# nathancunn/ParticleMDI.jl

Hardware: AMD Instinct MI355X
Metric: Gibbs iters/sec (and obs·particles/sec) at 1/2/4/8 GPUs vs CPU ref (higher is better)
Workload: dtype f64

## Files before the change

### particlemdi.jl_amd/csrc/pmdi_sweep2_body.h

```cpp
#pragma once
#include "pmdi_arith.h"
#include "pmdi_internal.h"
#include "pmdi_sweep2_layout.h"

#ifndef PM2_LANE_API_PROVIDED
#include "pmdi_wave.h"
#define PM2_DEV __device__ __forceinline__
#define PM2_COLD __device__ __noinline__
extern __shared__ __attribute__((aligned(16))) unsigned char pm2_smem_[];
#define PM2_SMEM (pm2_smem_)
#define PM2_TID() ((int)threadIdx.x)
#define PM2_BID() ((int)blockIdx.x)
#define PM2_BALLOT(p) __ballot(p)
#define PM2_SHFL64(v, src) pm2_shfl64((v), (src))
#define PM2_WAVE_BARRIER() do { __builtin_amdgcn_fence(__ATOMIC_ACQ_REL, "wavefront"); __builtin_amdgcn_wave_barrier(); } while (0)
#define PM2_BARRIER() __syncthreads()
#define PM2_LDS_BARRIER() asm volatile("s_waitcnt lgkmcnt(0)\n\ts_barrier" ::: "memory")
#define PM2_UNI(x) __builtin_amdgcn_readfirstlane(x)
#define PM2_CLOCK() ((long long)clock64())
#define PM2_WALLCLOCK() ((long long)wall_clock64())
#if defined(__HIP_DEVICE_COMPILE__)
#define PM2_G(T, p) ((__attribute__((address_space(1))) T *)(p))
#define PM2_CONST __attribute__((address_space(4)))
#ifdef PM2_NO_LAUNDER
// ... 931 lines not shown
                u64 wm0 = readlane_u64(wm, l0);
                const int base0 = readlane_i(base, l0), inpl0 = readlane_i(inpl, l0);
                int rnk = 0;
                while (wm0) {
                    const int ns = pm2_ffs64(wm0) - 1;
                    wm0 &= wm0 - 1;
                    if (ns != inpl0) {
                        const int newc = base0 + rnk - (inpl0 >= 0 ? 1 : 0);
                        const int t = v.tgt_get(v.tab_get(cs, ns));
                        if (lane < N) v.tab_set(newc, lane, lane == ns ? t : v.tab_get(cs, lane));
                    }
                    rnk += 1;
                }
                PM2_WAVE_BARRIER();
                if (inpl0 >= 0 && lane == 0) v.tab_set(cs, inpl0, v.tgt_get(v.tab_get(cs, inpl0)));
                if (lane == l0) todo = false;
            }
            }
            ncol_new += tot;
        }
        PM2_WAVE_BARRIER();
        PHC(6);
        unsigned mpr_r = INFU;
        int slot_r = 0;
        if (nk <= 64) {
            const u64 repb = PM2_BALLOT(rep_r);
            for (u64 rb = repb; rb; rb &= rb - 1) {
                const int j2 = pm2_ffs64(rb) - 1;
                const int v2 = readlane_i(kv_r, j2);
                const unsigned m2 = (unsigned)readlane_i((int)mp_r, j2);
                if (v2 == kv_r) mpr_r = m2;
            }
            for (u64 rb = repb; rb; rb &= rb - 1) {
                const int j2 = pm2_ffs64(rb) - 1;
                const unsigned m2 = (unsigned)readlane_i((int)mp_r, j2);
                if (m2 < mpr_r) ++slot_r;
            }
        }
        for (int j0 = 0; j0 < nk; j0 += 64) {
            const int j = j0 + lane;
            if (j < nk) {
                const int key = klist[j];
                const int v0 = kval[j];
                unsigned mpr = mpr_r;
                int slot = slot_r;
                if (nk > 64) {
                    int jr = j;
                    for (int j2 = 0; j2 < nk; ++j2) if (krep[j2] && kval[j2] == v0) jr = j2;
                    mpr = minp[klist[jr]];
                    slot = 0;
                    for (int j2 = 0; j2 < nk; ++j2) if (krep[j2] && minp[klist[j2]] < mpr) ++slot;
                }
                lds<u8>(v.base + L.knew)[key] = (u8)slot;
                if (krep[j]) {
                    const int pl = (int)(mpr >> 16), cl = (int)(mpr & 0xffffu);
                    const int ns = key - (key / N) * N;
                    const u64 wm = nclone ? v.wmask_get(cl) : 0ull;
                    int newc = cl;
                    if ((wm >> ns) & 1ull) {
                        const int bi = v.cbi_get(cl);
                        const int inpl = (bi & 0xff) - 1, base = bi >> 8;
                        const int rnk = pm2_popc64(wm & ((1ull << ns) - 1ull));
                        newc = (inpl >= 0) ? (ns == inpl ? cl : base + rnk - 1) : base + rnk;
                    }
                    lds<int>(v.base + L.clsval)[slot] = v0; lds<int>(v.base + L.clslead)[slot] = pl; lds<int>(v.base + L.leadcol)[slot] = newc;
                }
            }
        }
        PM2_WAVE_BARRIER();
        PHD(13);
        PHC(7);
        int ndefer = 0;
        {
            const bool on = lane < D && fl[lane];
            for (int e0 = 0; e0 < nd; e0 += 4) {
                int cj[4], nj[4], sj[4];
                bool mine[4];
                St stj[4];
                double gj[4];
#pragma unroll
                for (int j = 0; j < 4; ++j) {
                    cj[j] = 0; nj[j] = 0; sj[j] = NONE8; mine[j] = false;
                    if (e0 + j < nd) {
                        cj[j] = chosen(e0 + j);
                        sj[j] = v.slot_of(cj[j]);
                        mine[j] = sj[j] != NONE8 && v.tgt_get(cj[j]) == cj[j];
                        if (mine[j]) nj[j] = v.cn_get(cj[j]); else ndefer += 1;
                    }
                }
#pragma unroll
                for (int j = 0; j < 4; ++j) {
                    stj[j] = pf; gj[j] = 0.0;
                    if (mine[j]) {
                        if (e0 + j > 0) stj[j] = st_load(v, cj[j], x, lane < D);
                        if (lane == 0 && (GO || v.kind == K_GAUSSIAN)) gj[j] = PM2_G(const double, d.gtab)[nj[j]];
                    }
                }
#pragma unroll
                for (int j = 0; j < 4; ++j) {
                    if (mine[j]) {
                        st_add_store(v, cj[j], stj[j], x, nj[j], on);
                        cache_fill(v, k, sj[j], stj[j].a, stj[j].b, nj[j], false, true, gj[j]);
                    }
                }
            }
        }
        PHD(15);
        PHC(8);
        PM2_WAVE_BARRIER();
        for (int e0 = 0; e0 < nd; e0 += 64) {
            const int e = e0 + lane;
            if (e < nd) { const int c = chosen(e); v.ncop_set(c, 0); v.firstp_set(c, 0x7fffffff); }
        }
        for (int j0 = 0; j0 < nk; j0 += 64) { const int j = j0 + lane; if (j < nk) minp[klist[j]] = INFU; }
        for (int w = lane; w < P / 64 + 1; w += 64) { bmc[w] = 0; bmf[w] = 0; }
        if (lane == 0) {
            long long *st = stat();
            pm2_atomic_add((u64 *)&st[0], (u64)maxid);
            pm2_atomic_add((u64 *)&st[4], (u64)ncls);
            pm2_atomic_add((u64 *)&st[2], (u64)nclone);
            pm2_atomic_add((u64 *)&st[5], (u64)1);
            pm2_atomic_max((u64 *)&st[3], (u64)(maxid + nclone));
            long long *w_ = wk(k);
            w_[WK_EVAL] += dsc[DS_NNEED]; w_[WK_UPD] += nd; w_[WK_CLONE] += nclone; w_[WK_SPLITS] += ncol_new - ncol;
            dsc[DS_MAXID] = maxid + nclone; dsc[DS_NCLS] = nrep; dsc[DS_NCOL] = ncol_new; dsc[DS_NDX] = 0; dsc[DS_NCLONE] = nclone;
            dsc[DS_ND] = ndefer ? nd : 0; dsc[DS_NDLOW] = nd_low;
            dsc[DS_FOLLOW] = (nclone != 0 || ncls != 1 || nk != 1) ? 1 : 0;
            dsc[DS_DIRTY] = (nclone != 0 || ncls != 1 || nk != 1 || dsc[DS_CHANGED] != 0) ? 1 : 0;
            dsc[DS_CHANGED] = 0;
        }
        (void)pos;
        return true;
    }

    PM2_DEV bool help_stats(int i_cur)
    {
        constexpr int HB = 2;
        int item = 0;
        bool any = false;
#pragma nounroll
        for (int k = 0; k < K; ++k) {
            const DV v = view(k);
            const int *dsc = v.dsc();
            const int nd = PM2_UNI(dsc[DS_ND]);
            if (nd == 0) continue;
            any = true;
            const int nd_low = PM2_UNI(dsc[DS_NDLOW]);
            const auto &d = ap->ds[k];
            const int D = d.D;
            const u8 *fl = flk(k);
            const bool on = lane < D && fl[lane];
            const u16 *clist = lds<u16>(v.base + L.clist);
            auto sb = PM2_G(double, v.ar.sb());
            double x = 0.0;
            bool have_x = false;
            for (int e0 = 0; e0 < nd; e0 += HB, ++item) {
                if (item % NW != wave) continue;
                if (!have_x) { x = obs_x(k, i_cur); have_x = true; }
                int cj[HB], tj[HB], nj[HB];
                bool mine[HB];
                double sgj[HB], btj[HB];
#pragma unroll
                for (int j = 0; j < HB; ++j) {
                    cj[j] = 0; tj[j] = 0; nj[j] = 0; mine[j] = false;
                    if (e0 + j < nd) {
                        const int e = e0 + j;
                        cj[j] = (e < nd_low) ? (int)clist[e] : PM2_G(const int, v.ar.dl())[e - nd_low];
                        tj[j] = v.tgt_get(cj[j]);
                        mine[j] = !(v.slot_of(cj[j]) != NONE8 && tj[j] == cj[j]);
                        if (mine[j]) nj[j] = v.cn_get(tj[j]);
                    }
                }
                if ((GO || v.kind == K_GAUSSIAN)) {
#pragma unroll
                    for (int j = 0; j < HB; ++j) {
                        sgj[j] = 0.0; btj[j] = 0.5;
                        if (mine[j] && lane < D) { sgj[j] = sb[((size_t)cj[j] * D + lane) * 2]; btj[j] = sb[((size_t)cj[j] * D + lane) * 2 + 1]; }
                    }
#pragma unroll
                    for (int j = 0; j < HB; ++j) {
                        if (mine[j]) {
                            double sg = sgj[j], bt = btj[j];
                            if (on) pmdi_arith::gauss_add_sb(x, nj[j], sg, bt);
                            if (lane < D && (on || tj[j] != cj[j])) { sb[((size_t)tj[j] * D + lane) * 2] = sg; sb[((size_t)tj[j] * D + lane) * 2 + 1] = bt; }
                        }
                    }
                } else if ((!GO && v.kind == K_CATEGORICAL)) {
                    auto cn_ = PM2_G(int, v.ar.cnt());
                    const int Lc = v.Lc;
#pragma unroll
                    for (int j = 0; j < HB; ++j) {
                        if (mine[j] && lane < D) {
                            const size_t so = ((size_t)cj[j] * D + lane) * Lc, to = ((size_t)tj[j] * D + lane) * Lc;
                            const int xl = (int)x - 1;
                            const int cx = cn_[so + xl];
                            if (tj[j] != cj[j]) for (int l = 0; l < Lc; ++l) cn_[to + l] = cn_[so + l];
                            if (on) cn_[to + xl] = cx + 1;
                        }
                    }
                } else {
                    auto nb_ = PM2_G(long long, v.ar.nbs());
#pragma unroll
                    for (int j = 0; j < HB; ++j)
                        if (mine[j] && lane < D && (on || tj[j] != cj[j]))
                            nb_[(size_t)tj[j] * D + lane] = nb_[(size_t)cj[j] * D + lane] + (on ? (long long)x : 0ll);
                }
            }
        }
        return any;
    }

    PM2_DEV void census(const DV &v, bool active, int mult, int r, int cl, int ns, int c, int p)
    {
        int *dsc = v.dsc();
        const int key3 = ((r * P + cl) * N + ns) * 16 + mult;
        const u64 act = PM2_BALLOT(active);
        if (act == 0) return;
        const int l0 = pm2_ffs64(act) - 1;
        const int k0 = readlane_i(key3, l0);
        const bool uni = PM2_BALLOT(active && key3 == k0) == act;
        if (uni ? (lane == l0) : active) {
            const int cnt = uni ? pm2_popc64(act) * mult : mult;
            if (c < v.idcap) {
                pm2_atomic_add(lds<int>(v.base + L.ncop) + c, cnt);
                pm2_atomic_min(lds<int>(v.base + L.firstp) + c, p);
                pm2_atomic_or(lds<u64>(v.base + L.cbm) + (c >> 6), 1ull << (c & 63));
            } else {
                const int old = pm2_atomic_min(v.ar.firstp() + c, p);
                pm2_atomic_add(v.ar.ncop() + c, cnt);
                if (old == 0x7fffffff) { const int idx = pm2_atomic_add(&dsc[DS_NDX], 1); PM2_G(int, v.ar.dl())[idx] = c; }
            }
            const int key = r * N + ns;
            pm2_atomic_min(&lds<unsigned>(v.base + L.minp)[key], ((unsigned)p << 16) | (unsigned)cl);
            pm2_atomic_or(lds<u64>(v.base + L.kbm) + (key >> 6), 1ull << (key & 63));
            v.cmask_or(cl, 1ull << ns);
        }
    }

    PM2_DEV void cumsum_pairwise(const double (&w)[PPL], double (&c)[PPL])
    {
        constexpr int LPB = 64 / PPL;
        double sl[PPL];
#pragma unroll
        for (int u = 0; u < PPL; ++u) sl[u] = 0.0;
        const int blk = (tid * PPL) >> 6;
        const int lib = tid % LPB;
        double *tot = lds<double>(L.leaf_tot), *car = lds<double>(L.leaf_carry);
        double acc = 0.0;
        for (int pass = 0; pass < 2; ++pass) {
            const bool mine = (pass == 0) ? (blk != 1) : (blk == 1);
            double carry_in = 0.0;
            if (pass == 1) carry_in = tot[0];
            for (int t = 0; t < LPB; ++t) {
                const double cin = prev_lane_d(acc);
                if (mine && lib == t) {
                    double s = (t == 0) ? carry_in : cin;
#pragma unroll
                    for (int u = 0; u < PPL; ++u) {
                        const int p = tid * PPL + u;
                        if (p == 0) continue;
                        const bool first = (p == 1) || ((p & 63) == 0 && p >= 128);
                        s = first ? w[u] : s + w[u];
                        sl[u] = s;
                    }
                    acc = s;
                }
            }
            if (mine && lib == LPB - 1) tot[blk] = acc;
            PM2_BARRIER();
        }
        const int nb = P >> 6;
        double *lv = car;
        if (wave == 0) {
            if (tid == 0) lds<double>(L.red)[121] = w[0];
            for (int h = 1; (nb >> h) >= 2; ++h) {
                const int cnt = nb >> h, off = nb - (nb >> (h - 1)), offp = (h >= 2) ? nb - (nb >> (h - 2)) : 0;
                if (lane < cnt) {
                    double val;
                    if (h == 1) val = (lane == 0) ? tot[1] : tot[2 * lane] + tot[2 * lane + 1];
                    else val = lv[offp + 2 * lane] + lv[offp + 2 * lane + 1];
                    lv[off + lane] = val;
                }
                PM2_WAVE_BARRIER();
            }
        }
        PM2_BARRIER();
        double carry = lds<double>(L.red)[121];
        if (blk >= 2) {
            const int j = 32 - __builtin_clz((unsigned)blk);
            carry = carry + lv[nb - (nb >> (j - 2))];
            for (int h = j - 2; h >= 0; --h)
                if ((blk >> h) & 1) {
                    const int g = (blk >> h) - 1;
                    carry = carry + (h == 0 ? tot[g] : lv[nb - (nb >> (h - 1)) + g]);
                }
        }
#pragma unroll
        for (int u = 0; u < PPL; ++u) {
            const int p = tid * PPL + u;
            c[u] = (p == 0) ? w[u] : carry + sl[u];
        }
    }

    PM2_DEV void resample(long long pos, double mx)
    {
        PHR(0);
        double w[PPL];
#pragma unroll
        for (int u = 0; u < PPL; ++u) w[u] = exp(lw[u] - mx);
        const double u01 = pmdi_arith::uniform01<false>(seed, iter, (unsigned)pos, 0, 0, SITE_RESAMPLE_U);
        const double usl = pmdi_arith::uniform01<false>(seed, iter, (unsigned)pos, 0, 0, SITE_RESAMPLE_SLOT);
        double c[PPL];
        PHR(1);
        cumsum_pairwise(w, c);
        PHR(2);
        double *utab = lds<double>(L.tr);
        u16 *jtab = lds<u16>(L.tr + L.rs_jtab), *raw = lds<u16>(L.tr + L.rs_raw), *anc = lds<u16>(L.tr + L.rs_anc);
        double *red = lds<double>(L.red);
        if (tid == T - 1) red[0] = c[PPL - 1];
        {
            const double h = 1.0 / (double)P;
            const int j = tid * PPL;
            double u = pmdi_arith::resample_u_at(u01, P, j);
#pragma unroll
            for (int uu = 0; uu < PPL; ++uu) { utab[j + uu] = u; u = u + h; }
        }
        PM2_BARRIER();
        PHR(3);
        {
            const double last = red[0];
#pragma unroll
            for (int uu = 0; uu < PPL; ++uu) {
                const double q = c[uu] / last;
                int J = (int)((q - utab[0]) * (double)P) + 1;
                if (J < 0) J = 0;
                if (J > P) J = P;
                while (J < P && q >= utab[J]) ++J;
                while (J > 0 && !(q >= utab[J - 1])) --J;
                jtab[tid * PPL + uu] = (u16)J;
            }
        }
        PM2_BARRIER();
        PHR(4);
        {
            int lo = 0;
#pragma unroll
            for (int uu = 0; uu < PPL; ++uu) {
                const int j = tid * PPL + uu;
                if (uu == 0 || !((int)jtab[lo] > j)) {
                    int hi = P - 1;
                    while (lo < hi) { const int mid = (lo + hi) >> 1; if ((int)jtab[mid] > j) hi = mid; else lo = mid + 1; }
                }
                raw[j] = (u16)lo;
            }
        }
        int js = (int)(usl * (double)P);
        if (js >= P) js = P - 1;
        PM2_BARRIER();
        PHR(5);
#pragma unroll
        for (int uu = 0; uu < PPL; ++uu) {
            const int p = tid * PPL + uu;
            anc[p] = (p == 0) ? (u16)0 : (p <= js ? raw[p - 1] : raw[p]);
            lw.set(uu, 1.0);
        }
        PM2_BARRIER();
        u16 *scol = lds<u16>(L.tr), *mult = lds<u16>(L.tr + P * 2), *cmap = lds<u16>(L.tr + P * 4);
        u8 *scsl = lds<u8>(L.tr + P * 6);
        int *hist = lds<int>(L.tr + L.rs_hist);
#pragma nounroll
        for (int k = 0; k < K; ++k) {
            const DV v = view(k);
            int *dsc = v.dsc();
            const int ncol_old = dsc[DS_NCOL], oldmax = dsc[DS_MAXID], ncls_old = dsc[DS_NCLS];
            PHR(6);
            int ck[PPL], rk[PPL];
            col_get(k, ck);
#pragma unroll
            for (int uu = 0; uu < PPL; ++uu) rk[uu] = csl_get(k, uu);
#pragma unroll
            for (int uu = 0; uu < PPL; ++uu) { const int p = tid * PPL + uu; scol[p] = (u16)ck[uu]; scsl[p] = (u8)rk[uu]; }
            for (int e = tid; e < ncol_old; e += T) mult[e] = 0;
            for (int e = tid; e <= oldmax && e < v.idcap; e += T) hist[e] = 0;
            if (tid < CLSMAX) lds<int>(L.red)[RI_CLSMIN + tid] = 0x7fffffff;
            if (tid == 0) sc()[SC_TMP0] = 0;
            PM2_BARRIER();
#pragma unroll
            for (int uu = 0; uu < PPL; ++uu) {
                const int p = tid * PPL + uu;
                const int an = anc[p];
                ck[uu] = scol[an]; rk[uu] = scsl[an];
            }
            PHR(7);
#pragma unroll
            for (int uu = 0; uu < PPL; ++uu) {
                const int cl = ck[uu], r = rk[uu];
                bool start = true;
                if (uu > 0) start = cl != ck[uu - 1] || r != rk[uu - 1];
                int cnt = 1;
                {
                    bool go = true;
#pragma unroll
                    for (int u2 = uu + 1; u2 < PPL; ++u2) { go = go && ck[u2] == cl && rk[u2] == r; cnt += go ? 1 : 0; }
                }
                const u64 act = PM2_BALLOT(start);
                if (act) {
                    const int l0 = pm2_ffs64(act) - 1;
                    const int key = cl * CLSMAX + r;
                    const int key0 = readlane_i(key, l0);
                    const bool uni = PM2_BALLOT(start && key == key0) == act;
                    int tot = cnt;
                    if (uni) {
                        tot = 0;
#pragma unroll
                        for (int c_ = 1; c_ <= PPL; ++c_) tot += c_ * pm2_popc64(PM2_BALLOT(start && cnt == c_));
                    }
                    if (uni ? (lane == l0) : start) {
                        pm2_atomic_add((unsigned *)mult + (cl >> 1), (unsigned)tot << ((cl & 1) * 16));
                        pm2_atomic_min(&lds<int>(L.red)[RI_CLSMIN + r], tid * PPL + uu);
                    }
                }
            }
            PM2_BARRIER();
            PHR(8);
            int ncol_new = 0;
            for (int b = 0; b < ncol_old; b += T) {
                const int cc = b + tid;
                const bool live = cc < ncol_old && mult[cc] != 0;
                const u64 bal = PM2_BALLOT(live);
                if (lane == 0) lds<int>(L.red)[RI_WCNT + wave] = pm2_popc64(bal);
                PM2_BARRIER();
                int basew = ncol_new, tot = 0;
                for (int w_ = 0; w_ < T / 64; ++w_) { const int cnt = lds<int>(L.red)[RI_WCNT + w_]; if (w_ < wave) basew += cnt; tot += cnt; }
                if (live) cmap[cc] = (u16)(basew + pm2_popc64(bal & ((1ull << lane) - 1ull)));
                ncol_new += tot;
                PM2_BARRIER();
            }
            PHR(9);
            for (int idx = tid; idx < ncol_old * N; idx += T) {
                const int cc = idx / N;
                const int m = mult[cc];
                if (m) {
                    const int id = v.tab_get(cc, idx - cc * N);
                    if (id < v.idcap) pm2_atomic_add(&hist[id], m); else pm2_atomic_add(v.ar.ncop() + id, m);
                }
            }
            PM2_BARRIER();
            PHR(10);
            int newmax = 0;
            for (int b = 0; b < oldmax; b += T) {
                const int id = 1 + b + tid;
                int occ = 0;
                if (id <= oldmax) occ = (id < v.idcap) ? hist[id] : PM2_G(int, v.ar.ncop())[id];
                const bool live = occ != 0;
                const u64 bal = PM2_BALLOT(live);
                if (lane == 0) lds<int>(L.red)[RI_WCNT + wave] = pm2_popc64(bal);
                PM2_BARRIER();
                int basew = newmax, tot = 0;
                for (int w_ = 0; w_ < T / 64; ++w_) { const int cnt = lds<int>(L.red)[RI_WCNT + w_]; if (w_ < wave) basew += cnt; tot += cnt; }
                if (id <= oldmax) v.tgt_set(id, live ? basew + pm2_popc64(bal & ((1ull << lane) - 1ull)) + 1 : 0);
                newmax += tot;
                PM2_BARRIER();
            }
            PHR(11);
            for (int b = 0; b < oldmax; b += T) {
                const int id = 1 + b + tid;
                int nid = 0, occ = 0, cnv = 0;
                if (id <= oldmax) {
                    nid = v.tgt_get(id);
                    occ = (id < v.idcap) ? hist[id] : PM2_G(int, v.ar.ncop())[id];
                    cnv = v.cn_get(id);
                    if (id >= v.idcap) PM2_G(int, v.ar.ncop())[id] = 0;
                }
                {
                    const u64 mvb = PM2_BALLOT(nid != 0 && nid != id);
                    if (lane == 0 && mvb) pm2_atomic_add(&sc()[SC_TMP0], pm2_popc64(mvb));
                }
                PM2_BARRIER();
                if (id <= oldmax) {
                    if (nid) { v.counts_set(nid, occ); v.cn_set(nid, cnv); }
                    if (id > newmax) v.counts_set(id, 0);
                }
                PM2_BARRIER();
            }
            PHR(12);
            if (sc()[SC_TMP0] != 0) {
                const int D = ap->ds[k].D;
                if ((GO || v.kind == K_GAUSSIAN)) {
                    auto sb = PM2_G(double, v.ar.sb());
                    const long long nitems = (long long)oldmax * D;
                    for (long long b = 0; b < nitems; b += T) {
                        const long long it = b + tid;
                        const int id = 1 + (int)(it / D), q = (int)(it - (long long)(id - 1) * D);
                        const int nid = (it < nitems) ? v.tgt_get(id) : 0;
                        const bool mv = nid != 0 && nid != id;
                        double sg = 0.0, bt = 0.0;
                        if (mv) { sg = sb[((size_t)id * D + q) * 2]; bt = sb[((size_t)id * D + q) * 2 + 1]; }
                        PM2_BARRIER();
                        if (mv) { sb[((size_t)nid * D + q) * 2] = sg; sb[((size_t)nid * D + q) * 2 + 1] = bt; }
                    }
                } else if ((!GO && v.kind == K_CATEGORICAL)) {
                    auto cn_ = PM2_G(int, v.ar.cnt());
                    const int W = D * v.Lc;
                    const long long nitems = (long long)oldmax * W;
                    for (long long b = 0; b < nitems; b += T) {
                        const long long it = b + tid;
                        const int id = 1 + (int)(it / W), q = (int)(it - (long long)(id - 1) * W);
                        const int nid = (it < nitems) ? v.tgt_get(id) : 0;
                        const bool mv = nid != 0 && nid != id;
                        int c_ = 0;
                        if (mv) c_ = cn_[(size_t)id * W + q];
                        PM2_BARRIER();
                        if (mv) cn_[(size_t)nid * W + q] = c_;
                    }
                } else {
                    auto nb_ = PM2_G(long long, v.ar.nbs());
                    const long long nitems = (long long)oldmax * D;
                    for (long long b = 0; b < nitems; b += T) {
                        const long long it = b + tid;
                        const int id = 1 + (int)(it / D), q = (int)(it - (long long)(id - 1) * D);
                        const int nid = (it < nitems) ? v.tgt_get(id) : 0;
                        const bool mv = nid != 0 && nid != id;
                        long long S_ = 0;
                        if (mv) S_ = nb_[(size_t)id * D + q];
                        PM2_BARRIER();
                        if (mv) nb_[(size_t)nid * D + q] = S_;
                    }
                }
            }
            PM2_BARRIER();
            PHR(13);
            if (wave == k) {
                int *slot_id = lds<int>(v.base + L.slot_id);
                int olds = 0, news = 0;
                if (lane < NS) { olds = slot_id[lane]; news = olds ? v.tgt_get(olds) : 0; }
                PM2_WAVE_BARRIER();
                if (lane < NS && olds) v.slot_set(olds, NONE8);
                PM2_WAVE_BARRIER();
                if (lane < NS) { slot_id[lane] = news; if (news) v.slot_set(news, lane); }
            }
            {
                const int cpr = (2 * T) / N;
                for (int c0 = 0; c0 < ncol_old; c0 += cpr) {
                    int nv[2], dc[2], dn[2];
#pragma unroll
                    for (int h = 0; h < 2; ++h) {
                        const int idx = h * T + tid;
                        const int cc = c0 + idx / N, nn = idx - (idx / N) * N;
                        nv[h] = 0; dc[h] = -1; dn[h] = nn;
                        if (idx < cpr * N && cc < ncol_old && mult[cc] != 0) { nv[h] = v.tgt_get(v.tab_get(cc, nn)); dc[h] = cmap[cc]; }
                    }
                    PM2_BARRIER();
#pragma unroll
                    for (int h = 0; h < 2; ++h) if (dc[h] >= 0) v.tab_set(dc[h], dn[h], nv[h]);
                    PM2_BARRIER();
                }
            }
#pragma unroll
            for (int uu = 0; uu < PPL; ++uu) ck[uu] = cmap[ck[uu]];
            {
                int *redi = lds<int>(L.red);
                int nc2 = 0;
                for (int r = 0; r < ncls_old; ++r) nc2 += (redi[RI_CLSMIN + r] != 0x7fffffff) ? 1 : 0;
                if (tid < ncls_old) {
                    int s = 0;
                    const int mine = redi[RI_CLSMIN + tid];
                    for (int r2 = 0; r2 < ncls_old; ++r2) if (redi[RI_CLSMIN + r2] < mine) ++s;
                    redi[RI_NEWSLOT + tid] = s;
                    redi[RI_CLSVAL + tid] = lds<int>(v.base + L.clsval)[tid];
                }
                PM2_BARRIER();
#pragma unroll
                for (int uu = 0; uu < PPL; ++uu) {
                    const int p = tid * PPL + uu;
                    const int r = rk[uu];
                    const int ns_ = redi[RI_NEWSLOT + r];
                    rk[uu] = ns_;
                    if (redi[RI_CLSMIN + r] == p) {
                        lds<int>(v.base + L.clsval)[ns_] = redi[RI_CLSVAL + r]; lds<int>(v.base + L.clslead)[ns_] = p; lds<int>(v.base + L.leadcol)[ns_] = ck[uu];
                    }
                }
                col_put(k, ck);
#pragma unroll
                for (int uu = 0; uu < PPL; ++uu) csl_put(k, uu, rk[uu]);
                if (tid == 0) {
                    const int moved = sc()[SC_TMP0];
                    dsc[DS_NCLS] = nc2; dsc[DS_NCOL] = ncol_new; dsc[DS_MAXID] = newmax; dsc[DS_DIRTY] = 1;
                    long long *w_ = wk(k);
                    w_[WK_COLS] += ncol_old; w_[WK_MOVED] += moved; w_[WK_MOVE_EVENTS] += moved ? 1 : 0;
                }
            }
            PM2_BARRIER();
        }
        PHR(15);
    }

    PM2_DEV void run(const SweepArgs *ap_, int chain_)
    {
        ap = (const PM2_CONST SweepArgs *)ap_; chain = chain_;
        const auto &a = *ap;
        tid = PM2_TID(); lane = tid & 63; wave = tid >> 6;
        N = a.N; P = a.P; n = a.n; n1 = a.n1; iter = a.iter;
        seed = a.seed + (unsigned long long)chain;
        const long long t_start = PM2_CLOCK();
        const long long t_wall = a.phase ? PM2_WALLCLOCK() : 0ll;
        const bool owner = wave < K;
        auto order = PM2_G(const int, a.order) + (size_t)chain * n;
        auto logphi = PM2_G(const double, a.logphi) + (size_t)chain * a.npairs;
        if (tid < SC_COUNT) sc()[tid] = 0;
        if (tid < 8) stat()[tid] = 0;
        if (tid < KMAX2 * 8) lds<long long>(L.wk)[tid] = 0;
        if (tid < 16) lds<long long>(L.ph)[tid] = 0;
        long long ph_last = 0;
        int ph_cur = 0;
#ifdef PM2_DETAIL_TIMERS
        phd_last = PM2_CLOCK(); phd_cur = 15;
#define PH2(i_) do { } while (0)
#else
#define PH2(i_) do { if (a.phase && tid == 0) { const long long t_ = PM2_CLOCK(); lds<long long>(L.ph)[ph_cur] += t_ - ph_last; ph_last = t_; ph_cur = (i_); } } while (0)
#endif
        if (a.phase && tid == 0) ph_last = PM2_CLOCK();
        PM2_BARRIER();
#pragma unroll
        for (int u = 0; u < PPL; ++u) lw.set(u, a.lw_init);
#pragma unroll
        for (int k = 0; k < K; ++k)
#pragma unroll
            for (int j = 0; j < NCP; ++j) colp.set(k * NCP + j, 0u);
#pragma unroll
        for (int k = 0; k < NCSW; ++k) cslp.set(k, (csl_t)0);
#pragma unroll
        for (int s = 0; s < NS; ++s) { c_mu.set(s, 0.0); c_lam.set(s, 1.0); }
        PM2_BARRIER();
        if (owner) prefix(wave);
        PM2_BARRIER();
        PH2(1);

        double xnext = 0.0;
        int ns0_next = 0;
        int i_next = order[n1 - 1];
        int i_next2 = (n1 < n) ? order[n1] : 0;
        if (owner) {
            xnext = obs_x(wave, i_next);
            ns0_next = PM2_G(const int, a.s_in)[((size_t)chain * K + wave) * n + i_next];
        }
        pend_slot = -1; pend_g = 0.0;
        int failed = 0, handed = 0;
        long long pos_handed = 0;
        for (long long pos = n1 - 1; pos < n; ++pos) {
            PM2_LAUNDER(ap, SweepArgs);
            PM2_FRESH_VGPR(tid); PM2_FRESH_VGPR(lane);
            const double x = xnext;
            const int ns0_cur = ns0_next;
            const int i_cur = i_next;
            if (pos + 1 < n) {
                i_next = i_next2;
                if (owner) {
                    xnext = obs_x(wave, i_next);
                    ns0_next = PM2_G(const int, a.s_in)[((size_t)chain * K + wave) * n + i_next];
                }
                if (pos + 2 < n) i_next2 = order[pos + 2];
            }
            PH2(1);
            if (owner) phase_a(wave, x, ns0_cur, pos);
            PH2(2);
            PM2_BARRIER();
            PH2(3);
            if (sc()[SC_FAIL]) { failed = sc()[SC_FAIL]; break; }
            unsigned nsp[PPL];
#pragma unroll
            for (int u = 0; u < PPL; ++u) nsp[u] = 0;
#pragma nounroll
            for (int k = 0; k < K; ++k) {
                const DV v = view(k);
                const int ns0 = v.dsc()[DS_NS0];
                PHD(5);
                int cl_[PPL], r_[PPL], c_[PPL];
                RegArr<int, PPL> nsv;
                double inc_[PPL];
                bool draw_any = false;
#pragma unroll
                for (int u = 0; u < PPL; ++u) {
                    const int p = tid * PPL + u;
                    r_[u] = csl_get(k, u);
                    cl_[u] = (int)((colp[k * NCP + (u >> 1)] >> ((u & 1) * 16)) & 0xffffu);
                    const int hot = (int)cdf_get(v, r_[u], N + 1);
                    inc_[u] = cdf_get(v, r_[u], N);
                    const int ns = (p == 0) ? ns0 : hot;
                    nsv.set(u, ns);
                    draw_any |= ns < 0;
                }
                PHD(6);
                if (PM2_BALLOT(draw_any)) {
#pragma nounroll
                    for (int u = 0; u < PPL; ++u) {
                        if (nsv[u] < 0) {
                            const int p = tid * PPL + u;
                            const int rr = csl_get(k, u);
                            const double u01 = pmdi_arith::uniform01<false>(seed, iter, (unsigned)pos, (unsigned)k, (unsigned)p, SITE_DRAW);
                            int ns = 0, t = 0;
                            if (!CDFA || rr < v.cdfl) {
                                const double *row = v.cdf_row_l(rr);
                                for (; t + 4 <= N - 1; t += 4) {
                                    const double a0 = row[t], a1 = row[t + 1], a2 = row[t + 2], a3 = row[t + 3];
                                    ns += ((a0 > u01) ? 0 : 1) + ((a1 > u01) ? 0 : 1) + ((a2 > u01) ? 0 : 1) + ((a3 > u01) ? 0 : 1);
                                }
                                for (; t < N - 1; ++t) ns += (row[t] > u01) ? 0 : 1;
                            } else {
                                auto row = PM2_G(const double, v.ar.cdfg()) + (size_t)rr * (N + 2);
                                for (; t < N - 1; ++t) ns += (row[t] > u01) ? 0 : 1;
                            }
                            nsv.set(u, ns);
                        }
                    }
                }
                PHD(7);
                unsigned packed = 0;
#pragma unroll
                for (int u = 0; u < PPL; ++u) {
                    const int ns = nsv[u];
                    lw.set(u, lw[u] + inc_[u]);
                    c_[u] = v.tab_get(cl_[u], ns);
                    nsp[u] |= (unsigned)ns << (8 * k);
                    packed |= (unsigned)ns << (8 * (u & 3));
                    if ((u & 3) == 3 || u == PPL - 1) {
                        u8 *ss = v.ar.sstar() + (size_t)pos * P + (size_t)tid * PPL + (u & ~3);
                        if (PPL >= 4) *PM2_G(unsigned, ss) = packed;
                        else if (PPL == 2) *PM2_G(u16, ss) = (u16)packed;
                        else *PM2_G(u8, ss) = (u8)packed;
                        packed = 0;
                    }
                }
                PHD(8);
                {
                    int keyu[PPL];
#pragma unroll
                    for (int u = 0; u < PPL; ++u) keyu[u] = (r_[u] * P + cl_[u]) * N + nsv[u];
                    bool allsame = true;
#pragma unroll
                    for (int u = 1; u < PPL; ++u) allsame = allsame && keyu[u] == keyu[0];
                    if (PM2_BALLOT(!allsame) == 0) {
                        census(v, true, PPL, r_[0], cl_[0], nsv[0], c_[0], tid * PPL);
                    } else {
#pragma unroll
                        for (int u = 0; u < PPL; ++u) {
                            bool dup = false;
                            int mult = 0;
#pragma unroll
                            for (int u2 = 0; u2 < PPL; ++u2) {
                                const bool same = keyu[u2] == keyu[u];
                                if (u2 < u) dup |= same;
                                if (u2 >= u) mult += same ? 1 : 0;
                            }
                            census(v, !dup, mult, r_[u], cl_[u], nsv[u], c_[u], tid * PPL + u);
                        }
                    }
                }
            }
            PHD(9);
            if (K > 1) {
#pragma unroll
                for (int u = 0; u < PPL; ++u) {
                    int pr = 0;
                    double wv_ = lw[u];
#pragma unroll
                    for (int k1 = 0; k1 < K - 1; ++k1)
#pragma unroll
                        for (int k2 = k1 + 1; k2 < K; ++k2) {
                            wv_ += (((nsp[u] >> (8 * k1)) & 0xffu) == ((nsp[u] >> (8 * k2)) & 0xffu)) ? logphi[pr] : 0.0;
                            ++pr;
                        }
                    lw.set(u, wv_);
                }
            }
            double *red = lds<double>(L.red);
            {
                double mx = lw[0], mn = lw[0];
#pragma unroll
                for (int u = 1; u < PPL; ++u) { mx = (lw[u] > mx) ? lw[u] : mx; mn = (lw[u] < mn) ? lw[u] : mn; }
                mx = wave_max_d(mx); mn = wave_min_d(mn);
                if (lane == 0) { red[RD_MAX + wave] = mx; red[RD_MIN + wave] = mn; }
            }
            PH2(4);
            PM2_BARRIER();
            PH2(5);
            double mx = red[RD_MAX], mn = red[RD_MIN];
            for (int w_ = 1; w_ < NW; ++w_) { mx = (red[RD_MAX + w_] > mx) ? red[RD_MAX + w_] : mx; mn = (red[RD_MIN + w_] < mn) ? red[RD_MIN + w_] : mn; }
            PHD(10);
            const bool lw_flat = mx == mn;
            if (!lw_flat) {
                double sa = 0.0, sq = 0.0;
#pragma nounroll
                for (int u = 0; u < PPL; ++u) { const double w = exp(lw_get(u) - mx); sa += w; sq += w * w; }
                sa = wave_sum_d(sa); sq = wave_sum_d(sq);
                if (lane == 0) { red[RD_SA + wave] = sa; red[RD_SQ + wave] = sq; }
            }
            if (owner) phase_c(wave, x, pos);
            PHC(9);
            PH2(6);
            PM2_BARRIER();
            PHC(15);
            PH2(7);
            int fcode = sc()[SC_FAIL];
            if (fcode && sc()[SC_TMP2]) fcode = 1;
            if (fcode && (fcode == 1 || !a.resume)) { failed = fcode; break; }
            if (help_stats(i_cur)) PM2_BARRIER();
#pragma nounroll
            for (int k = 0; k < K; ++k) {
                const DV v = view(k);
                if (!v.dsc()[DS_FOLLOW]) continue;
                const bool cloned = v.dsc()[DS_NCLONE] != 0;
                int ck[PPL];
                col_get(k, ck);
#pragma unroll
                for (int u = 0; u < PPL; ++u) {
                    const int cl = ck[u], ns = (int)((nsp[u] >> (8 * k)) & 0xffu);
                    const u64 wm = cloned ? v.wmask_get(cl) : 0ull;
                    if ((wm >> ns) & 1ull) {
                        const int bi = v.cbi_get(cl);
                        const int inpl = (bi & 0xff) - 1, base = bi >> 8;
                        const int rnk = pm2_popc64(wm & ((1ull << ns) - 1ull));
                        ck[u] = (inpl >= 0) ? (ns == inpl ? cl : base + rnk - 1) : base + rnk;
                    }
                    csl_put(k, u, (int)lds<u8>(v.base + L.knew)[csl_get(k, u) * N + ns]);
                }
                col_put(k, ck);
            }
            if (__builtin_expect(fcode != 0, 0)) { handed = fcode; pos_handed = pos; break; }
            double ess = (double)P;
            if (!lw_flat) {
                double sa = 0.0, sq = 0.0;
                for (int w_ = 0; w_ < NW; ++w_) { sa += red[RD_SA + w_]; sq += red[RD_SQ + w_]; }
                ess = (sa * sa) / sq;
            }
            if (pmdi_arith::ess_needs_sequential_redo(ess, P)) {
                double *wt = lds<double>(L.tr);
                PM2_BARRIER();
#pragma unroll
                for (int u = 0; u < PPL; ++u) wt[tid * PPL + u] = exp(lw[u] - mx);
                PM2_BARRIER();
                if (tid == 0) {
                    double na = 0.0, nb = 0.0;
                    for (int p = 0; p < P; ++p) { na += wt[p]; nb += wt[p] * wt[p]; }
                    red[120] = (na * na) / nb;
                }
                PM2_BARRIER();
                ess = red[120];
                PM2_BARRIER();
            }
            const bool res = pmdi_arith::ess_resamples(ess, P);
            if (res) {
                PH2(8);
                if (tid == 0) stat()[1] += 1;
                resample(pos, mx);
                PH2(7);
            }
            if (a.trace_on && tid == 0) {
                auto tr = PM2_G(double, a.trace) + ((size_t)chain * (n - n1 + 1) + (pos - (n1 - 1))) * (2 + 2 * K);
                tr[0] = ess; tr[1] = res ? 1.0 : 0.0;
                for (int k = 0; k < K; ++k) { tr[2 + k] = (double)view(k).dsc()[DS_MAXID]; tr[2 + K + k] = (double)view(k).dsc()[DS_NCLS]; }
            }
        }
        if (handed) {
            hand_over_cold(*this, pos_handed, handed, t_start);
#ifdef PM2_RESUME_GENERAL
            __builtin_amdgcn_fence(__ATOMIC_SEQ_CST, "agent");
            PM2_BARRIER();
            PM2_RESUME_GENERAL(K, NW, ap_);
#endif
            return;
        }
        if (failed) {
            if (tid == 0) {
                if (failed == 1) PM2_G(int, a.err)[chain] = -4;
                else if (a.requeue) {
                    PM2_G(int, a.requeue)[chain] = 1;
                    if (!a.err_keep) PM2_G(int, a.err)[chain] = 0;
                    if (a.handed) PM2_G(int, a.handed)[chain] = a.sweep_no;
                    if (a.requeue_total) {
                        pm2_atomic_add((u64 *)a.requeue_total + 3, (u64)1); pm2_atomic_add((u64 *)a.requeue_total + 2, (u64)1);
                        if (failed == 4 && sc()[SC_TMP1] > 2 * CLS) pm2_atomic_add((u64 *)a.requeue_total + 1, (u64)1);
                    }
                }
                else PM2_G(int, a.err)[chain] = PMDI_S2_REQUEUE;
                for (int e = 0; e < 8; ++e) PM2_G(long long, a.stats)[(size_t)chain * 8 + e] = 0;
                PM2_G(long long, a.stats)[(size_t)chain * 8 + 7] = (a.requeue && failed != 1) ? 0 : failed;
                PM2_G(long long, a.cost)[chain] = PM2_CLOCK() - t_start;
            }
            if (failed == 1) {
// ... 155 lines not shown
```

### particlemdi.jl_amd/csrc/pmdi_sweep2_layout.h

```cpp
#pragma once
#include "pmdi_internal.h"

#ifndef PM2_HD
#define PM2_HD inline __host__ __device__
#endif

namespace pmdi_s2 {

constexpr int NWMAX = 8;
#ifndef PM2_NS
#define PM2_NS 8
#endif
constexpr int NS = PM2_NS;
constexpr int XR = 4;
#ifndef PM2_XCAP
#define PM2_XCAP 24
#endif
constexpr int XCAP = PM2_XCAP;
constexpr int NR = (NS > 2 * XR) ? NS : 2 * XR;
constexpr int CLSMAX = 32;
PM2_HD constexpr int class_slot_bits(int K, int PPL, int NW) { return (K == 4 && PPL == 4 && NW == 4) ? 4 : 5; }
PM2_HD constexpr int class_slots_max(int K, int PPL, int NW) { return 1 << class_slot_bits(K, PPL, NW); }
PM2_HD constexpr bool cdf_rows_in_arena(int NW) { return NW > 4; }
constexpr int KCAPMAX = 256;
constexpr int RI_CLSMIN = 64, RI_NEWSLOT = 96, RI_CLSVAL = 128;
constexpr int RI_WCNT = 160;
constexpr int RD_MAX = 0, RD_MIN = NWMAX, RD_SA = 2 * NWMAX, RD_SQ = 3 * NWMAX;
constexpr int KMAX2 = 4;
constexpr int NONE8 = 0xFF;
constexpr unsigned INFU = 0xFFFFFFFFu;
constexpr int PMDI_S2_REQUEUE = 1;

enum { DS_MAXID = 0, DS_NCLS, DS_NCOL, DS_NDX, DS_ND, DS_NS0, DS_NX, DS_NNEED, DS_NCLONE, DS_NFLAG, DS_FOLLOW, DS_DIRTY, DS_NEEDMASK, DS_CHANGED, DS_NDLOW, DS_HALT, DS_COUNT = 16 };
enum { SC_FAIL = 0, SC_RES, SC_PSTAR, SC_NLEAF, SC_NPROG, SC_JS, SC_TMP0, SC_TMP1, SC_TMP2, SC_TMP3, SC_COUNT = 16 };

typedef S2Layout Layout;

PM2_HD void make_layout(int K, int N, int P, int Dmax, int cols_l, int idcap, int cls, int cdfl, Layout &L)
{
    const int CLS = cls;
    const int kcap = (CLS * N < KCAPMAX) ? CLS * N : KCAPMAX;
    if (cdfl > cls) cdfl = cls;
    L.cls = cls; L.kcap = kcap; L.cdfl = cdfl;
    int o = 0;
    auto take = [&](int bytes) { const int at = o; o = (o + bytes + 15) & ~15; return at; };
    const int Dp = (Dmax + 1) & ~1;
    L.Dp = Dp; L.cols_l = cols_l; L.idcap = idcap;
    L.red = take(128 * 8);
    L.sc = take(SC_COUNT * 4);
    L.stat = take(8 * 8);
    L.wk = take(KMAX2 * 8 * 8);
    L.ph = take(16 * 8);
    L.leaf_i1 = 0; L.leaf_n = 0; L.leaf_prog = 0;
    L.leaf_tot = take(64 * 8); L.leaf_carry = take(64 * 8);
    L.xfl = take(KMAX2 * 64);
    L.tr_tb = 0;
    L.tr_cdf = 128 * 8;
    L.tr_stride = L.tr_cdf + cdfl * (N + 2) * 8;
    if (L.tr_stride < NR * Dp * 8) L.tr_stride = NR * Dp * 8;
    L.tr_stride = (L.tr_stride + 15) & ~15;
    L.rs_jtab = P * 8; L.rs_raw = P * 10; L.rs_anc = P * 12; L.rs_hist = P * 14;
    const int rs = P * 14 + idcap * 4 + 64;
    int trb = K * L.tr_stride;
    if (trb < rs) trb = rs;
    L.tr_bytes = trb;
    L.tr = take(trb);
    const int b0 = o;
    o = 0;
    L.tab = take(cols_l * N * 2);
    L.cmask = take(cols_l * 8); L.wmask = take(cols_l * 8); L.cbi = take(cols_l * 4);
    L.counts = take(idcap * 4); L.cn = take(idcap * 4); L.ncop = take(idcap * 4); L.firstp = take(idcap * 4); L.tgt = take(idcap * 4);
    L.slotmap = take(idcap);
    L.ta = take(NS * Dp * 8); L.tax = L.ta;
    L.lp = take((NS + XCAP) * 8);
    L.slot_id = take(NS * 4); L.slot_cn = take(NS * 4); L.slot_g = take(NS * 8);
    L.clsval = take(CLS * 4); L.clslead = take(CLS * 4); L.leadcol = take(CLS * 4);
    L.minp = take(CLS * N * 4); L.nidv = take(CLS * N * 2); L.knew = take(CLS * N); L.itemj = take(CLS * N * 2);
    L.clist = take(idcap * 2); L.klist = take(kcap * 2); L.kval = take(kcap * 2); L.krep = take(kcap);
    L.bmc = take((P / 64 + 1) * 8); L.bmf = take((P / 64 + 1) * 8);
    L.cbm = take(((idcap + 63) / 64) * 8); L.kbm = take(((CLS * N + 63) / 64) * 8);
    L.xid = take(XCAP * 4);
    L.dsc = take(DS_COUNT * 4);
    L.ds_stride = o;
    L.ds0 = b0;
    L.total = b0 + K * L.ds_stride;
}

struct Shape { int nw, ppl; };
PM2_HD constexpr Shape shape_for(int P)
{
    return P == 256 ? Shape{4, 1} : P == 512 ? Shape{4, 2} : P == 1024 ? Shape{4, 4} : P == 2048 ? Shape{8, 4} : Shape{0, 0};
}
PM2_HD constexpr Shape shape_for(int K, int P) { return (K >= 1 && K <= KMAX2) ? shape_for(P) : Shape{0, 0}; }

}

inline void pmdi_sweep2_layout(int K, int N, int P, int Dmax, int cols_l, int idcap, int cls, int cdfl, S2Layout *L)
{
    pmdi_s2::make_layout(K, N, P, Dmax, cols_l, idcap, cls, cdfl, *L);
}
inline int pmdi_sweep2_threads(int K, int P) { return 64 * pmdi_s2::shape_for(K, P).nw; }
inline int pmdi_sweep2_max_classes(int K, int P)
{
    const pmdi_s2::Shape s = pmdi_s2::shape_for(K, P);
    return s.nw ? pmdi_s2::class_slots_max(K, s.ppl, s.nw) : 0;
}
inline bool pmdi_sweep2_cdf_arena(int K, int P)
{
    const pmdi_s2::Shape s = pmdi_s2::shape_for(K, P);
    return s.nw && pmdi_s2::cdf_rows_in_arena(s.nw);
}
inline bool pmdi_sweep2_supports(int K, int N, int P, int Dmax, long long cap)
{
    (void)cap;
    return N >= 2 && N <= 64 && Dmax <= 64 && pmdi_s2::shape_for(K, P).nw != 0;
}
```

Baseline: 890.2.

## Restructure resample ancestor computation and fuse cluster-id compaction with row moves

Resampling now finds ancestors by counting how many systematic-resample points fall in each particle's bin with LDS atomics, then taking an exclusive scan. This replaces the write-jtab, barrier, binary-search sequence. The id-compaction pass is merged with the counts/cn update and the parameter-row move loop, and the rows to move are batched four per thread per barrier. The last column-compaction block is overlapped with the histogram pass, and the relabel and slot-update passes are skipped when nothing moved. The goal is fewer block barriers and serial LDS searches per resample. The cost is more complex bookkeeping and extra LDS slots in the reduction area.

```diff
diff --git a/particlemdi.jl_amd/csrc/pmdi_sweep2_body.h b/particlemdi.jl_amd/csrc/pmdi_sweep2_body.h
--- a/particlemdi.jl_amd/csrc/pmdi_sweep2_body.h
+++ b/particlemdi.jl_amd/csrc/pmdi_sweep2_body.h
@@ -1257,6 +1257,35 @@
         }
     }
 
+    template <int WPI, class GP>
+    PM2_DEV void move_rows(GP g, int W, int cnt, int nid0, const int *src)
+    {
+        const int nitems = cnt * W;
+        for (int b = 0; b < nitems; b += 4 * T) {
+            decltype(g[0] + g[0]) val[4][WPI];
+            long long dst[4];
+#pragma unroll
+            for (int r = 0; r < 4; ++r) {
+                const int it = b + r * T + tid;
+                dst[r] = -1;
+                if (it < nitems) {
+                    const int j = it / W, q = it - j * W;
+                    const size_t so = ((size_t)src[j] * W + q) * WPI;
+                    dst[r] = (long long)(((size_t)(nid0 + j) * W + q) * WPI);
+#pragma unroll
+                    for (int w_ = 0; w_ < WPI; ++w_) val[r][w_] = g[so + w_];
+                }
+            }
+            PM2_BARRIER();
+#pragma unroll
+            for (int r = 0; r < 4; ++r)
+                if (dst[r] >= 0) {
+#pragma unroll
+                    for (int w_ = 0; w_ < WPI; ++w_) g[(size_t)dst[r] + w_] = val[r][w_];
+                }
+        }
+    }
+
     PM2_DEV void resample(long long pos, double mx)
     {
         PHR(0);
@@ -1270,54 +1299,93 @@
         cumsum_pairwise(w, c);
         PHR(2);
         double *utab = lds<double>(L.tr);
-        u16 *jtab = lds<u16>(L.tr + L.rs_jtab), *raw = lds<u16>(L.tr + L.rs_raw), *anc = lds<u16>(L.tr + L.rs_anc);
+        u16 *nown = lds<u16>(L.tr + L.rs_jtab), *anc = lds<u16>(L.tr + L.rs_anc);
         double *red = lds<double>(L.red);
+        int *redi = lds<int>(L.red);
         if (tid == T - 1) red[0] = c[PPL - 1];
         {
             const double h = 1.0 / (double)P;
             const int j = tid * PPL;
             double u = pmdi_arith::resample_u_at(u01, P, j);
 #pragma unroll
-            for (int uu = 0; uu < PPL; ++uu) { utab[j + uu] = u; u = u + h; }
-        }
+            for (int uu = 0; uu < PPL; ++uu) { utab[j + uu] = u; nown[j + uu] = 0; u = u + h; }
+        }
+        if (tid < NW) redi[RI_WBASE + tid] = 0;
         PM2_BARRIER();
         PHR(3);
+        int J[PPL];
         {
-            const double last = red[0];
+            const double last = red[0], u0 = utab[0];
+            double q[PPL];
 #pragma unroll
             for (int uu = 0; uu < PPL; ++uu) {
-                const double q = c[uu] / last;
-                int J = (int)((q - utab[0]) * (double)P) + 1;
-                if (J < 0) J = 0;
-                if (J > P) J = P;
-                while (J < P && q >= utab[J]) ++J;
-                while (J > 0 && !(q >= utab[J - 1])) --J;
-                jtab[tid * PPL + uu] = (u16)J;
-            }
-        }
-        PM2_BARRIER();
+                q[uu] = c[uu] / last;
+                int g = (int)((q[uu] - u0) * (double)P) + 1;
+                if (g < 0) g = 0;
+                if (g > P) g = P;
+                J[uu] = g;
+            }
+            bool moving = true;
+            while (moving) {
+                double ua[PPL], ub[PPL];
+#pragma unroll
+                for (int uu = 0; uu < PPL; ++uu) {
+                    ua[uu] = (J[uu] < P) ? utab[J[uu]] : 0.0;
+                    ub[uu] = (J[uu] > 0) ? utab[J[uu] - 1] : 0.0;
+                }
+                moving = false;
+#pragma unroll
+                for (int uu = 0; uu < PPL; ++uu) {
+                    const bool up = J[uu] < P && q[uu] >= ua[uu];
+                    const bool dn = !up && J[uu] > 0 && !(q[uu] >= ub[uu]);
+                    J[uu] += (up ? 1 : 0) - (dn ? 1 : 0);
+                    moving = moving || up || dn;
+                }
+            }
+        }
         PHR(4);
         {
-            int lo = 0;
 #pragma unroll
             for (int uu = 0; uu < PPL; ++uu) {
-                const int j = tid * PPL + uu;
-                if (uu == 0 || !((int)jtab[lo] > j)) {
-                    int hi = P - 1;
-                    while (lo < hi) { const int mid = (lo + hi) >> 1; if ((int)jtab[mid] > j) hi = mid; else lo = mid + 1; }
-                }
-                raw[j] = (u16)lo;
+                int cnt = 1;
+                bool start = true;
+                if (uu > 0) start = J[uu] != J[uu - 1];
+                {
+                    bool go = true;
+#pragma unroll
+                    for (int u2 = uu + 1; u2 < PPL; ++u2) { go = go && J[u2] == J[uu]; cnt += go ? 1 : 0; }
+                }
+                if (start && J[uu] < P) pm2_atomic_add((unsigned *)nown + (J[uu] >> 1), (unsigned)cnt << ((J[uu] & 1) * 16));
+            }
+#pragma unroll
+            for (int w_ = 1; w_ < NW; ++w_) {
+                int below = 0;
+#pragma unroll
+                for (int uu = 0; uu < PPL; ++uu) below += pm2_popc64(PM2_BALLOT(J[uu] < w_ * 64 * PPL));
+                if (lane == 0 && below) pm2_atomic_add(&redi[RI_WBASE + w_], below);
             }
         }
         int js = (int)(usl * (double)P);
         if (js >= P) js = P - 1;
         PM2_BARRIER();
         PHR(5);
-#pragma unroll
-        for (int uu = 0; uu < PPL; ++uu) {
-            const int p = tid * PPL + uu;
-            anc[p] = (p == 0) ? (u16)0 : (p <= js ? raw[p - 1] : raw[p]);
-            lw.set(uu, 1.0);
+        {
+            int own[PPL + 1];
+            int tot_ = 0, run = 0;
+#pragma unroll
+            for (int uu = 0; uu < PPL; ++uu) { run += (int)nown[tid * PPL + uu]; own[uu + 1] = run; }
+            const int ex = redi[RI_WBASE + wave] + wave_excl_scan_i(run, tot_);
+            own[0] = ex;
+#pragma unroll
+            for (int uu = 0; uu < PPL; ++uu) own[uu + 1] += ex;
+#pragma unroll
+            for (int uu = 0; uu <= PPL; ++uu) if (own[uu] > P - 1) own[uu] = P - 1;
+#pragma unroll
+            for (int uu = 0; uu < PPL; ++uu) {
+                const int p = tid * PPL + uu;
+                anc[p] = (p == 0) ? (u16)0 : (u16)(p <= js ? own[uu] : own[uu + 1]);
+                lw.set(uu, 1.0);
+            }
         }
         PM2_BARRIER();
         u16 *scol = lds<u16>(L.tr), *mult = lds<u16>(L.tr + P * 2), *cmap = lds<u16>(L.tr + P * 4);
@@ -1379,18 +1447,23 @@
             PM2_BARRIER();
             PHR(8);
             int ncol_new = 0;
-            for (int b = 0; b < ncol_old; b += T) {
+            const int cb_last = ncol_old > 0 ? ((ncol_old - 1) / T) * T : 0;
+            for (int b = 0; b < cb_last; b += T) {
                 const int cc = b + tid;
-                const bool live = cc < ncol_old && mult[cc] != 0;
+                const bool live = mult[cc] != 0;
                 const u64 bal = PM2_BALLOT(live);
-                if (lane == 0) lds<int>(L.red)[RI_WCNT + wave] = pm2_popc64(bal);
+                if (lane == 0) redi[RI_WCNTC + wave] = pm2_popc64(bal);
                 PM2_BARRIER();
                 int basew = ncol_new, tot = 0;
-                for (int w_ = 0; w_ < T / 64; ++w_) { const int cnt = lds<int>(L.red)[RI_WCNT + w_]; if (w_ < wave) basew += cnt; tot += cnt; }
+                for (int w_ = 0; w_ < T / 64; ++w_) { const int cnt = redi[RI_WCNTC + w_]; if (w_ < wave) basew += cnt; tot += cnt; }
                 if (live) cmap[cc] = (u16)(basew + pm2_popc64(bal & ((1ull << lane) - 1ull)));
                 ncol_new += tot;
                 PM2_BARRIER();
             }
+            const int ccl = cb_last + tid;
+            const bool livec = ccl < ncol_old && mult[ccl] != 0;
+            const u64 balc = PM2_BALLOT(livec);
+            if (lane == 0) redi[RI_WCNTC + wave] = pm2_popc64(balc);
             PHR(9);
             for (int idx = tid; idx < ncol_old * N; idx += T) {
                 const int cc = idx / N;
@@ -1401,91 +1474,57 @@
                 }
             }
             PM2_BARRIER();
-            PHR(10);
-            int newmax = 0;
-            for (int b = 0; b < oldmax; b += T) {
+            {
+                int basew = ncol_new, tot = 0;
+                for (int w_ = 0; w_ < T / 64; ++w_) { const int cnt = redi[RI_WCNTC + w_]; if (w_ < wave) basew += cnt; tot += cnt; }
+                if (livec) cmap[ccl] = (u16)(basew + pm2_popc64(balc & ((1ull << lane) - 1ull)));
+                ncol_new += tot;
+            }
+            int newmax = 0, moved = 0;
+            int *src = lds<int>(L.tr + L.rs_jtab);
+            for (int b = 0; b < oldmax || b == 0; b += T) {
+                PHR(10);
                 const int id = 1 + b + tid;
                 int occ = 0;
                 if (id <= oldmax) occ = (id < v.idcap) ? hist[id] : PM2_G(int, v.ar.ncop())[id];
                 const bool live = occ != 0;
                 const u64 bal = PM2_BALLOT(live);
-                if (lane == 0) lds<int>(L.red)[RI_WCNT + wave] = pm2_popc64(bal);
+                if (lane == 0) redi[RI_WCNTI + wave] = pm2_popc64(bal);
                 PM2_BARRIER();
+                PHR(11);
                 int basew = newmax, tot = 0;
-                for (int w_ = 0; w_ < T / 64; ++w_) { const int cnt = lds<int>(L.red)[RI_WCNT + w_]; if (w_ < wave) basew += cnt; tot += cnt; }
-                if (id <= oldmax) v.tgt_set(id, live ? basew + pm2_popc64(bal & ((1ull << lane) - 1ull)) + 1 : 0);
-                newmax += tot;
-                PM2_BARRIER();
-            }
-            PHR(11);
-            for (int b = 0; b < oldmax; b += T) {
-                const int id = 1 + b + tid;
-                int nid = 0, occ = 0, cnv = 0;
+                for (int w_ = 0; w_ < T / 64; ++w_) { const int cnt = redi[RI_WCNTI + w_]; if (w_ < wave) basew += cnt; tot += cnt; }
+                const int nid = live ? basew + pm2_popc64(bal & ((1ull << lane) - 1ull)) + 1 : 0;
+                int cnv = 0;
                 if (id <= oldmax) {
-                    nid = v.tgt_get(id);
-                    occ = (id < v.idcap) ? hist[id] : PM2_G(int, v.ar.ncop())[id];
+                    v.tgt_set(id, nid);
                     cnv = v.cn_get(id);
                     if (id >= v.idcap) PM2_G(int, v.ar.ncop())[id] = 0;
                 }
+                const bool mv = nid != 0 && nid != id;
                 {
-                    const u64 mvb = PM2_BALLOT(nid != 0 && nid != id);
+                    const u64 mvb = PM2_BALLOT(mv);
                     if (lane == 0 && mvb) pm2_atomic_add(&sc()[SC_TMP0], pm2_popc64(mvb));
                 }
+                if (mv) src[nid - newmax - 1] = id;
                 PM2_BARRIER();
-                if (id <= oldmax) {
-                    if (nid) { v.counts_set(nid, occ); v.cn_set(nid, cnv); }
-                    if (id > newmax) v.counts_set(id, 0);
-                }
-                PM2_BARRIER();
-            }
-            PHR(12);
-            if (sc()[SC_TMP0] != 0) {
-                const int D = ap->ds[k].D;
-                if ((GO || v.kind == K_GAUSSIAN)) {
-                    auto sb = PM2_G(double, v.ar.sb());
-                    const long long nitems = (long long)oldmax * D;
-                    for (long long b = 0; b < nitems; b += T) {
-                        const long long it = b + tid;
-                        const int id = 1 + (int)(it / D), q = (int)(it - (long long)(id - 1) * D);
-                        const int nid = (it < nitems) ? v.tgt_get(id) : 0;
-                        const bool mv = nid != 0 && nid != id;
-                        double sg = 0.0, bt = 0.0;
-                        if (mv) { sg = sb[((size_t)id * D + q) * 2]; bt = sb[((size_t)id * D + q) * 2 + 1]; }
-                        PM2_BARRIER();
-                        if (mv) { sb[((size_t)nid * D + q) * 2] = sg; sb[((size_t)nid * D + q) * 2 + 1] = bt; }
-                    }
-                } else if ((!GO && v.kind == K_CATEGORICAL)) {
-                    auto cn_ = PM2_G(int, v.ar.cnt());
-                    const int W = D * v.Lc;
-                    const long long nitems = (long long)oldmax * W;
-                    for (long long b = 0; b < nitems; b += T) {
-                        const long long it = b + tid;
-                        const int id = 1 + (int)(it / W), q = (int)(it - (long long)(id - 1) * W);
-                        const int nid = (it < nitems) ? v.tgt_get(id) : 0;
-                        const bool mv = nid != 0 && nid != id;
-                        int c_ = 0;
-                        if (mv) c_ = cn_[(size_t)id * W + q];
-                        PM2_BARRIER();
-                        if (mv) cn_[(size_t)nid * W + q] = c_;
-                    }
-                } else {
-                    auto nb_ = PM2_G(long long, v.ar.nbs());
-                    const long long nitems = (long long)oldmax * D;
-                    for (long long b = 0; b < nitems; b += T) {
-                        const long long it = b + tid;
-                        const int id = 1 + (int)(it / D), q = (int)(it - (long long)(id - 1) * D);
-                        const int nid = (it < nitems) ? v.tgt_get(id) : 0;
-                        const bool mv = nid != 0 && nid != id;
-                        long long S_ = 0;
-                        if (mv) S_ = nb_[(size_t)id * D + q];
-                        PM2_BARRIER();
-                        if (mv) nb_[(size_t)nid * D + q] = S_;
-                    }
-                }
-            }
-            PM2_BARRIER();
+                if (nid) { v.counts_set(nid, occ); v.cn_set(nid, cnv); }
+                const int mvall = sc()[SC_TMP0], mvr = mvall - moved;
+                moved = mvall;
+                PHR(12);
+                if (mvr != 0) {
+                    const int D = ap->ds[k].D;
+                    const int nid0 = newmax + tot - mvr + 1;
+                    const int *srcb = src + (tot - mvr);
+                    if ((GO || v.kind == K_GAUSSIAN)) move_rows<2>(PM2_G(double, v.ar.sb()), D, mvr, nid0, srcb);
+                    else if ((!GO && v.kind == K_CATEGORICAL)) move_rows<1>(PM2_G(int, v.ar.cnt()), D * v.Lc, mvr, nid0, srcb);
+                    else move_rows<1>(PM2_G(long long, v.ar.nbs()), D, mvr, nid0, srcb);
+                }
+                newmax += tot;
+            }
+            for (int id = newmax + 1 + tid; id <= oldmax; id += T) v.counts_set(id, 0);
             PHR(13);
-            if (wave == k) {
+            if ((moved != 0 || newmax != oldmax) && wave == k) {
                 int *slot_id = lds<int>(v.base + L.slot_id);
                 int olds = 0, news = 0;
                 if (lane < NS) { olds = slot_id[lane]; news = olds ? v.tgt_get(olds) : 0; }
@@ -1494,7 +1533,7 @@
                 PM2_WAVE_BARRIER();
                 if (lane < NS) { slot_id[lane] = news; if (news) v.slot_set(news, lane); }
             }
-            {
+            if (moved != 0 || ncol_new != ncol_old) {
                 const int cpr = (2 * T) / N;
                 for (int c0 = 0; c0 < ncol_old; c0 += cpr) {
                     int nv[2], dc[2], dn[2];
@@ -1503,7 +1542,7 @@
                         const int idx = h * T + tid;
                         const int cc = c0 + idx / N, nn = idx - (idx / N) * N;
                         nv[h] = 0; dc[h] = -1; dn[h] = nn;
-                        if (idx < cpr * N && cc < ncol_old && mult[cc] != 0) { nv[h] = v.tgt_get(v.tab_get(cc, nn)); dc[h] = cmap[cc]; }
+                        if (idx < cpr * N && cc < ncol_old && mult[cc] != 0) { nv[h] = v.tab_get(cc, nn); if (moved != 0) nv[h] = v.tgt_get(nv[h]); dc[h] = cmap[cc]; }
                     }
                     PM2_BARRIER();
 #pragma unroll
@@ -1539,7 +1578,6 @@
 #pragma unroll
                 for (int uu = 0; uu < PPL; ++uu) csl_put(k, uu, rk[uu]);
                 if (tid == 0) {
-                    const int moved = sc()[SC_TMP0];
                     dsc[DS_NCLS] = nc2; dsc[DS_NCOL] = ncol_new; dsc[DS_MAXID] = newmax; dsc[DS_DIRTY] = 1;
                     long long *w_ = wk(k);
                     w_[WK_COLS] += ncol_old; w_[WK_MOVED] += moved; w_[WK_MOVE_EVENTS] += moved ? 1 : 0;
diff --git a/particlemdi.jl_amd/csrc/pmdi_sweep2_layout.h b/particlemdi.jl_amd/csrc/pmdi_sweep2_layout.h
--- a/particlemdi.jl_amd/csrc/pmdi_sweep2_layout.h
+++ b/particlemdi.jl_amd/csrc/pmdi_sweep2_layout.h
@@ -25,6 +25,8 @@
 constexpr int KCAPMAX = 256;
 constexpr int RI_CLSMIN = 64, RI_NEWSLOT = 96, RI_CLSVAL = 128;
 constexpr int RI_WCNT = 160;
+constexpr int RI_WBASE = 168;
+constexpr int RI_WCNTC = 176, RI_WCNTI = 184;
 constexpr int RD_MAX = 0, RD_MIN = NWMAX, RD_SA = 2 * NWMAX, RD_SQ = 3 * NWMAX;
 constexpr int KMAX2 = 4;
 constexpr int NONE8 = 0xFF;
```

After: 900.2, median of 6. +1.1%, better.
